# mike-gimelfarb/bboptpy

Measured on AMD Instinct MI355X. Metric: candidate-evals/sec, higher is better.
Workload: dtype f64; 1 GPU; ActiveCMAES n=128 np=4096 rosenbrock, 256 independent populations per GPU in lockstep; populations_per_gpu=256, n=128, np=4096, objective=rosenbrock

## Files before the change

### bboptpy_amd/csrc/bbo_cma.hip

```cpp
#include "bbo_cma_kernels.hpp"
#include "bbo_sep_kernels.hpp"
#include "bbo_chol_kernels.hpp"
#include "bbo_eig_mw.hpp"

#include <algorithm>
#include <atomic>
#include <cmath>
#include <cstdlib>
#include <limits>

namespace bbo {

namespace {

enum { K_SAMPLE = 0, K_RANK, K_WHITEN, K_GRAM, K_PATHS, K_COV, K_EIGEN, K_POST, K_STOP, K_COUNT };
static const char *const K_NAMES[K_COUNT] = { "bbo:cma_sample_eval", "bbo:cma_rank", "bbo:cma_whiten", "bbo:cma_gram", "bbo:cma_paths", "bbo:cma_cov", "bbo:cma_eigen", "bbo:cma_post", "bbo:cma_history_stop" };

int pick_maxt(int ld)
{
    const int per_wave = ((ld >> 4) + 3) / 4;
    if (per_wave <= 1) return 1;
    if (per_wave <= 2) return 2;
    if (per_wave <= 4) return 4;
    return 8;
// ... 487 lines not shown
    timer_.end(stream_);
    BBO_HIP(hipGetLastError());
    c_.use_zn = (zn_valid && !c.bound) ? 1 : 0;
}

void CmaEngine::launch_rank()
{
    const CmaConst &c = c_;
    rank_wrote_norms_ = false;
    timer_.begin(stream_, K_RANK);
    if (c.lambda <= 64 && c.lambda >= 2 && c.npop >= 4) {
        hipLaunchKernelGGL(cma_rank_wave, dim3((c.npop + 3) / 4), dim3(256), 0, stream_, d_, c_);
    } else if (c.lambda <= SORT_LDS_MAX && c.npop >= 4) {
        int m = 2;
        while (m < c.lambda) m <<= 1;
        allow_lds((const void*) cma_rank_sort, 128 * 1024);
        const size_t lds = rank_sort_merges(m, d_.dbg) ? (size_t) m * 24 : (size_t) std::max(m, 1024) * 12;
        hipLaunchKernelGGL(cma_rank_sort, dim3(c.npop), dim3(sort_threads(m)), lds, stream_, d_,
                c_, m);
        rank_wrote_norms_ = c.variant == 1 && c.use_zn && !basis_maybe_stale_;
    } else {
        if ((long) c.npop * ((c.lambda + 31) / 32) <= 256 && c.lambda >= 2048 && !(d_.dbg & (128 | 4096)))
            hipLaunchKernelGGL(cma_rank64, dim3((c.lambda + 3) / 4, c.npop), dim3(256), 0, stream_, d_, c_);
        else if ((long) c.npop * ((c.lambda + 31) / 32) <= 512 && c.lambda >= 512 && !(d_.dbg & 128))
            hipLaunchKernelGGL(cma_rank32, dim3((c.lambda + 7) / 8, c.npop), dim3(256), 0, stream_, d_, c_);
        else
            hipLaunchKernelGGL(cma_rank, dim3((c.lambda + 31) / 32, c.npop), dim3(256), 0, stream_, d_, c_);
        rank_wrote_norms_ = c.variant == 1 && c.use_zn && !basis_maybe_stale_;
    }
    timer_.end(stream_);
    BBO_HIP(hipGetLastError());
}

void CmaEngine::launch_update()
{
    const CmaConst &c = c_;
    if (c.variant == 3) {
        timer_.begin(stream_, K_PATHS);
        hipLaunchKernelGGL(chol_paths, dim3(c.npop), dim3(256), 0, stream_, d_, c_);
        timer_.end(stream_);
        const int NT = c.ld / 16;
        timer_.begin(stream_, K_GRAM);
        hipLaunchKernelGGL(chol_cprime, dim3(NT * (NT + 1) / 2, c.npop), dim3(256), 0, stream_, d_, c_);
        timer_.end(stream_);
        const int in_lds = c.ld <= 128 ? 1 : 0;
        const size_t lds = in_lds ? (size_t) c.ld * (c.ld + 1) * sizeof(double) : 0;
        timer_.begin(stream_, K_COV);
        hipLaunchKernelGGL(chol_factor, dim3(c.npop), dim3(256), lds, stream_, d_, c_, in_lds);
        timer_.end(stream_);
        BBO_HIP(hipGetLastError());
        return;
    }
    if (c.variant == 2) {
        timer_.begin(stream_, K_GRAM);
        hipLaunchKernelGGL(sep_moments, dim3(c.splits, (c.ld + 511) / 512, c.npop), dim3(256), 0,
                stream_, d_, c_);
        timer_.end(stream_);
        timer_.begin(stream_, K_PATHS);
        hipLaunchKernelGGL(sep_paths, dim3(c.npop), dim3(256), 0, stream_, d_, c_);
        timer_.end(stream_);
        BBO_HIP(hipGetLastError());
        return;
    }
    const bool norms_done = rank_wrote_norms_;
    rank_wrote_norms_ = false;
    if (c.variant == 1 && !norms_done) {
        timer_.begin(stream_, K_WHITEN);
// ... 18 lines not shown
        timer_.end(stream_);
        BBO_HIP(hipGetLastError());
    }
    if (c.ld == 128) {
        const size_t lds = (size_t) (2 * G128_CH * G128_LDY + 4 * G128_CH) * sizeof(double);
        allow_lds((const void*) cma_gram128, 80 * 1024);
        timer_.begin(stream_, K_GRAM);
        if (d_.dbg & 512)
            hipLaunchKernelGGL(cma_gram128, dim3(c.splits, c.npop), dim3(256), lds, stream_, d_, c_);
        else
            hipLaunchKernelGGL(cma_gram128s, dim3(c.splits, c.npop), dim3(256), 0, stream_, d_, c_);
        timer_.end(stream_);
        BBO_HIP(hipGetLastError());
    } else {
        const int NT = c.ld / 16, LT = NT * (NT + 1) / 2;
        const int ldy = gram_ldy(c.ld);
        dim3 grid(c.splits, (LT + 4 * GRAM_TPW - 1) / (4 * GRAM_TPW), c.npop);
        const size_t lds = gram_lds_bytes(c.ld, c.rps);
        allow_lds((const void*) cma_gram, (int) GRAM_LDS_MAX);
        timer_.begin(stream_, K_GRAM);
        hipLaunchKernelGGL(cma_gram, grid, dim3(256), lds, stream_, d_, c_, ldy);
        timer_.end(stream_);
        BBO_HIP(hipGetLastError());
    }
    timer_.begin(stream_, K_PATHS);
    if (c.lazy_isc && c.n >= 64 && !(d_.dbg & 131072))
        hipLaunchKernelGGL(cma_paths_lazy1k, dim3(c.npop), dim3(1024), 0, stream_, d_, c_);
    else if (c.lazy_isc)
        hipLaunchKernelGGL(cma_paths_lazy, dim3(c.npop), dim3(256), 0, stream_, d_, c_);
    else
        hipLaunchKernelGGL(cma_paths, dim3(c.npop), dim3(256), 0, stream_, d_, c_);
    timer_.end(stream_);
    BBO_HIP(hipGetLastError());
    {
        const int total = c.n * (c.n + 1) / 2;
        dim3 grid((total + 255) / 256, c.npop);
        timer_.begin(stream_, K_COV);
        hipLaunchKernelGGL(cma_cov, grid, dim3(256), 0, stream_, d_, c_);
        timer_.end(stream_);
        BBO_HIP(hipGetLastError());
    }
}

int CmaEngine::next_mw_xcd()
{
    static std::atomic<int> counter { 0 };
    return counter.fetch_add(1) & 7;
}

void CmaEngine::launch_eigen()
{
    const CmaConst &c = c_;
    if (c.variant >= 2) return;
    const EigPlan pl_lds = eig_plan(c.n, c.ld);
    const bool split128 = pl_lds.use_lds && pl_lds.threads == 512 && pl_lds.dc && c.npop <= split_maxp_
            && !(d_.dbg & (2 | 4 | 8 | 1024 | 4194304));
    const EigPlan pl = split128 ? eig_plan_split(c.n, c.ld) : pl_lds;
    bool wy4_packs = false, fcols_closed = false;
    allow_lds((const void*) cma_eigen, 160 * 1024 - 768);
    allow_lds((const void*) cma_eigen_g, 160 * 1024 - 768);
    allow_lds((const void*) cma_eigen_b, 160 * 1024 - 768);
    allow_lds((const void*) cma_eigen_256, 160 * 1024 - 768);
    allow_lds((const void*) cma_eigen_128, 160 * 1024 - 768);
    timer_.begin(stream_, K_EIGEN);
    const bool big_spread = c.n > 256 && pl.dc && !pl.hybrid && !mw_disabled_
            && !(d_.dbg & (2 | 16777216)) && mw_reserve((long) c.npop * 16);
    const bool small = c.n <= 16 && c.n >= 2 && c.ld == 16 && !(d_.dbg & 16);
    const int eig_path_bits = 1 | 2 | 4 | 8 | 1024 | 2048 | 8192 | 16384 | 32768 | 524288 | 2097152 | 4194304 | 8388608;
    const bool fixed_shape = c.n == 128 && c.ld == 128 && pl_lds.use_lds && pl_lds.dc && pl_lds.reg_path
            && pl_lds.threads == 512 && pl_lds.lda == EIG_FX_PLAN.lda && pl_lds.rc == EIG_FX_PLAN.rc
            && pl_lds.lds_bytes == EIG_FX_PLAN.lds_bytes && !d_.stamps && !(d_.dbg & eig_path_bits);
    const bool fixed128 = fixed_shape && c.npop > split_maxp_ && !split128 && c.lazy_isc;
    const bool fixed_r1 = fixed_shape && split128 && pl.hybrid;
    eig_fixed_last_ = (fixed128 || fixed_r1) && !small;
    if (small)
        hipLaunchKernelGGL(cma_eigen_small, dim3((c.npop + 3) / 4), dim3(256), 0, stream_, d_, c_, 0,
                1);
    else if (pl.threads == 128)
        hipLaunchKernelGGL(cma_eigen_128, dim3(c.npop), dim3(128), pl.lds_bytes, stream_, d_, c_,
                pl, 0);
    else if (pl.threads == 256)
        hipLaunchKernelGGL(cma_eigen_256, dim3(c.npop), dim3(256), pl.lds_bytes, stream_, d_, c_,
                pl, 0);
    else if (fixed128) {
        allow_lds((const void*) cma_eigen_fx128, 160 * 1024 - 768);
        const EigFxArgs fa { d_.C, d_.B, d_.D, d_.BDp, d_.eig_work, d_.scal, c.eigenfreq, c.honor_stop };
        hipLaunchKernelGGL(cma_eigen_fx128, dim3(c.npop), dim3(512), EIG_FX_PLAN.lds_bytes, stream_, fa);
    } else if (pl.use_lds)
        hipLaunchKernelGGL(cma_eigen, dim3(c.npop), dim3(512), pl.lds_bytes, stream_, d_, c_,
                pl, 0);
    else if (pl.hybrid && !(d_.dbg & (2 | 1024 | 4194304))) {
        const EigPlan plh = eig_plan(128, 128);
        allow_lds((const void*) cma_eigen_g1, 160 * 1024 - 768);
        allow_lds((const void*) cma_eigen_g2, 160 * 1024 - 768);
        allow_lds((const void*) cma_eig_halves, 160 * 1024 - 768);
        const bool use_mw = !split128 && !mw_disabled_ && !(d_.dbg & 16777216) && mw_reserve((long) c.npop * MW_G);
        if (split128 && fixed_r1) {
            allow_lds((const void*) cma_eigen_r1_fx128, 160 * 1024 - 768);
            const EigFxArgs fa { d_.C, d_.B, d_.D, d_.BDp, d_.eig_work, d_.scal, c.eigenfreq, c.honor_stop };
            hipLaunchKernelGGL(cma_eigen_r1_fx128, dim3(c.npop), dim3(512), EIG_FX_PLAN.lds_bytes, stream_, fa);
        } else if (split128) {
            allow_lds((const void*) cma_eigen_r1, 160 * 1024 - 768);
            hipLaunchKernelGGL(cma_eigen_r1, dim3(c.npop), dim3(512), pl_lds.lds_bytes, stream_, d_, c_,
                    pl_lds, 0);
        } else if (use_mw) {
            mw_launched_ = true;
            if (mw_buf_.count != (size_t) c.npop * MW_BUF_DOUBLES) mw_buf_.alloc((size_t) c.npop * MW_BUF_DOUBLES);
            const int istop = (d_.dbg & 536870912) ? 1 : 128;
            hipLaunchKernelGGL(cma_tred_mw, dim3(8 * MW_G, c.npop), dim3(MW_T), 0, stream_, d_, c_, 0,
                    mw_buf_.p, ++mw_launch_, istop, mw_xcd_);
            if (istop > 1) {
                allow_lds((const void*) cma_tred_tail, 160 * 1024 - 768);
                hipLaunchKernelGGL(cma_tred_tail, dim3(c.npop), dim3(512), pl.lds_bytes, stream_, d_, c_, pl, 0);
            }
        } else
            hipLaunchKernelGGL(cma_eigen_g1, dim3(c.npop), dim3(512), pl.lds_bytes, stream_, d_, c_, pl, 0);
        hipLaunchKernelGGL(cma_eig_halves, dim3(3, c.npop), dim3(512), plh.lds_bytes, stream_, d_, c_,
                plh, pl.lda);
        if ((long) c.npop * 8 <= 256 && !(d_.dbg & 67108864)) {
            hipLaunchKernelGGL(cma_eigen_g2, dim3(c.npop), dim3(512), pl.lds_bytes, stream_, d_, c_, pl, 1);
            hipLaunchKernelGGL(cma_eig_secular, dim3((c.n + 31) / 32, c.npop), dim3(512), 0, stream_, d_, c_);
            fcols_closed = !(c.n & 1) && c.lazy_isc && (long) c.npop * ((c.n + 15) / 16) <= 256
                    && !(d_.dbg & (33554432 | 134217728));
            if (fcols_closed) {
                hipLaunchKernelGGL(cma_eig_lowner, dim3((c.n + 31) / 32, c.npop), dim3(512), 0, stream_, d_, c_);
                hipLaunchKernelGGL(cma_eig_fcols, dim3((c.n + 31) / 32, c.npop), dim3(512), 0, stream_, d_, c_);
            } else
                hipLaunchKernelGGL(cma_eigen_g2, dim3(c.npop), dim3(512), pl.lds_bytes, stream_, d_, c_, pl, 2);
        } else
            hipLaunchKernelGGL(cma_eigen_g2, dim3(c.npop), dim3(512), pl.lds_bytes, stream_, d_, c_, pl, 0);
    } else if (pl.hybrid)
        hipLaunchKernelGGL(cma_eigen_g, dim3(c.npop), dim3(512), pl.lds_bytes, stream_, d_, c_,
// ... 90 lines not shown
    const CmaConst &c = c_;
    return c.variant < 2 && c.ld == 16 && c.n >= 2 && c.lambda_pad <= 64 && obj_.fused()
            && c.npop <= SMALL_FUSED_MAXP && !timer_.on() && !(d_.dbg & (16 | 64));
}

void CmaEngine::launch_small(int gens, bool honor_stop)
{
    c_.honor_stop = honor_stop ? 1 : 0;
    c_.use_zn = c_.bound ? 0 : 1;
    const int ldy = gram_ldy(c_.ld);
    size_t lds = gram_lds_bytes(c_.ld, c_.rps);
    lds = std::max(lds, (size_t) 64 * (c_.ld + 2) * sizeof(double));
    lds = std::max(lds, (size_t) (16 * (c_.ld + 2) + 64) * sizeof(double));
    const int scratch = (int) ((lds + 15) / 16 * 2);
    const size_t total = ((size_t) scratch + small_state_doubles(c_)) * sizeof(double);
    allow_lds((const void*) cma_small_generations, 120 * 1024);
    BBO_REQUIRE(total <= 120 * 1024, "small fused path: state does not fit LDS");
    hipLaunchKernelGGL(cma_small_generations, dim3(c_.npop), dim3(256), total, stream_, d_, c_,
            gens, ldy, scratch);
    BBO_HIP(hipGetLastError());
}

void CmaEngine::generation(bool honor_stop)
{
    if (small_fused_ok()) {
        launch_small(1, honor_stop);
        return;
    }
    c_.honor_stop = honor_stop ? 1 : 0;
    launch_sample_eval();
    if (obj_.needs_host()) host_evaluate();
    else if (obj_.is_program()) program_evaluate();
    launch_rank();
    launch_update();
    launch_eigen();
    launch_history_stop();
}

void CmaEngine::phase(int which)
{
    BBO_REQUIRE(inited_, "phase before init");
    BBO_HIP(hipSetDevice(params_.device));
    c_.honor_stop = 0;
    d_.mw_fault = mw_fault_from_env();
    switch (which) {
    case BBO_PHASE_SAMPLE_EVALUATE:
        launch_sample_eval();
        if (obj_.needs_host()) host_evaluate();
        else if (obj_.is_program()) program_evaluate();
        break;
    case BBO_PHASE_RANK: launch_rank(); break;
    case BBO_PHASE_UPDATE: launch_update(); break;
    case BBO_PHASE_EIGEN: launch_eigen(); break;
    case BBO_PHASE_HISTORY_STOP: launch_history_stop(); break;
    default: throw Error(BBO_ERR_ARG, "unknown CMA phase");
    }
    BBO_HIP(hipStreamSynchronize(stream_));
    if (mw_check_failed() && which == BBO_PHASE_EIGEN) {
        launch_eigen();
        BBO_HIP(hipStreamSynchronize(stream_));
    }
    timer_.collect();
    prog_timer_.collect();
}

void CmaEngine::inject_normals(const double *z, int count)
{
    BBO_REQUIRE(inited_, "inject_normals before init");
// ... 188 lines not shown
    if (k == "best_hist" || k == "kth_hist") {
        if (out && cap >= c.hlen)
            (k == "best_hist" ? hist_best_ : hist_kth_).download(out, c.hlen, (size_t) p * c.hlen);
        return c.hlen;
    }
    CmaScal s;
    scal_.download(&s, 1, p);
    if (k == "sigma") return o.one(s.sigma);
    if (k == "it") return o.one(s.it);
    if (k == "fev") return o.one(s.fev);
    if (k == "flag") return o.one(s.flag);
    if (k == "stop") return o.one(s.stop);
    if (k == "hsig") return o.one(s.hsig);
    if (k == "pslen") return o.one(s.pslen);
    if (k == "fbest") return o.one(s.fbest);
    if (k == "fworst") return o.one(s.fworst);
    if (k == "eigenlastev") return o.one(s.eigenlastev);
    if (k == "eigen_done") return o.one(s.eigen_done);
    if (k == "basis_ok") return o.one(s.basis_ok);
    if (k == "eig_stage") return o.one(s.eig_stage);
    if (k == "eig_mw_fail") return o.one(s.eig_mw_fail);
    if (k == "chol_repairs") {
        if (c.variant != 3) throw Error(BBO_ERR_KEY, "'chol_repairs' belongs to CholeskyCMAES");
        int r = 0;
        chol_repairs_.download(&r, 1, p);
        return o.one(r);
    }
    if (c.variant == 3 && k == "chol_tri") return o.one(chol_tri_ ? 1 : 0);
    if (c.variant == 3 && k == "stol") return o.one(c.stol);
    if (c.variant == 3 && k == "ranked") return o.one(c.ranked);
    if (k == "eig_mw_off") return o.one(mw_disabled_ ? 1 : 0);
    if (k == "eig_split_maxp") return o.one(split_maxp_);
    if (k == "eig_fixed128") return o.one(eig_fixed_last_ ? 1 : 0);
    if (k == "eig_mw_reserved") return o.one((double) mw_reserved_);
    if (k == "eig_mw_capacity") {
        MwBudget &b = MwBudget::get();
        std::lock_guard<std::mutex> lock(b.m);
        return o.one((double) b.capacity(params_.device));
    }
    if (k == "best_len") return o.one(s.hist_len);
    if (k == "best_buffer") return o.one(s.hist_head);
    if (k == "ibest") return o.one(s.ibw[0]);
    if (k == "n") return o.one(c.n);
    if (k == "lambda") return o.one(c.lambda);
    if (k == "mu") return o.one(c.mu);
    if (k == "mueff") return o.one(c.mueff);
    if (k == "cc") return o.one(c.cc);
    if (k == "cs") return o.one(c.cs);
    if (k == "c1") return o.one(c.c1);
    if (k == "cmu") return o.one(c.cmu);
    if (k == "cneg") return o.one(c.cneg);
    if (k == "alphaold") return o.one(c.alphaold);
    if (k == "cm") return o.one(c.cm);
    if (k == "ccov") return o.one(c.ccov);
    if (k == "damps") return o.one(c.damps);
    if (k == "chi") return o.one(c.chi);
    if (k == "eigenfreq") return o.one(c.eigenfreq);
    if (k == "hlen") return o.one(c.hlen);
    if (k == "ik") return o.one(c.ik);
    if (k == "mit") return o.one(c.mit);
    if (k == "mfev") return o.one(c.mfev);
    if (k == "sigma0") return o.one(c.sigma0);
    throw Error(BBO_ERR_KEY, "unknown state key '" + k + "'");
}

int CmaEngine::set(const std::string &k, int p, const double *in, int count)
// ... 147 lines not shown
```

### bboptpy_amd/csrc/bbo_cma.hpp

```cpp
#pragma once

#include "bbo_engine.hpp"

namespace bbo {

struct CmaScal {
    double sigma;
    double fbest, fworst;
    double pslen;
    double ybw[4];
    int ibw[4];
    int it, fev;
    int flag;
    int stop;
    int hsig;
    int eigenlastev, eigen_done;
    int hist_head, hist_len;
    int basis_ok;
    int eig_stage;
    int eig_mw_fail;
};

struct CmaConst {
    int n, ld;
// ... 59 lines not shown
    void optimize(int n, const double *lower, const double *upper, const double *guess,
            const ObjectiveSpec &obj, double *x_out, int *n_evals, int *converged) override;
    int get(const std::string &key, int population, double *out, int cap) override;
    int set(const std::string &key, int population, const double *in, int count) override;
    int dimension() const override { return c_.n; }

    void set_params(int np, double sigma, int mfev);
    void phase(int which);
    void inject_normals(const double *z, int count);
    double evaluate_point(const double *x);
    int lambda() const { return params_.np; }
    int populations() const { return params_.populations; }
    uint64_t seed() const { return params_.seed; }
    void set_seed(uint64_t s) { params_.seed = s; }
    void fresh_start(uint64_t s)
    {
        params_.seed = s;
        keep_bc_ = false;
    }

private:
    static const bbo_params &checked(const bbo_params &p);
    void generation(bool honor_stop) override;
    bool budget_spent(const CmaScal &s) const override { return s.fev >= c_.mfev; }
    void inspect(const std::vector<CmaScal> &sc) override;
    int chunk_limit(int want) override;
    void launch_chunk(int gens) override;
    void after_chunk(bool in_run) override;
    bool small_fused_ok() const;
    void launch_small(int gens, bool honor_stop);
    void launch_sample_eval();
    void launch_post(int mode);
    void launch_rank();
    void launch_update();
    void launch_eigen();
    void launch_history_stop();
    void host_evaluate();
    void program_evaluate();

    CmaConst c_ {};
    CmaDev d_ {};
    bool keep_bc_ = false;
    bool basis_maybe_stale_ = false;
    DevBuf<double> mw_buf_;
    unsigned long long mw_launch_ = 0;
    bool mw_disabled_ = false;
    int mw_xcd_ = next_mw_xcd();
    static int next_mw_xcd();
    long sample_wide_max_tiles_ = 512;
    long sample128_min_rows_ = 256 * 128;
    bool chol_tri_ = true;
    int split_maxp_ = 32;
    bool eig_fixed_last_ = false;
    bool rank_wrote_norms_ = false;
    int last_n_ = -1;

    DevBuf<double> zn2_, csep_, A_;
    DevBuf<double> X_, f_, xmean_, xold_, pc_, ps_, C_, B_, D_, isc_, BDp_, ISp_, S_,
            gram_part_, mean_part_, hist_best_, hist_kth_, eig_work_, weights_, zinject_, zrecord_;
    DevBuf<int> rank_, order_, chol_repairs_;
    DevBuf<long long> stamps_;
    int *mw_fail_host_ = nullptr;
    long mw_reserved_ = 0;
    bool mw_launched_ = false;
    bool mw_reserve(long workgroups);
    void mw_release();
    bool mw_check_failed();
};

}
```

### bboptpy_amd/csrc/bbo_cma_kernels.hpp

```cpp
#pragma once

#include "bbo_cma.hpp"
#include "bbo_objectives.hpp"
#include "bbo_rng.hpp"
#include "bbo_eig.hpp"
#include "bbo_rank.hpp"

namespace bbo {

typedef double d4_t __attribute__((ext_vector_type(4)));

#define BBO_INF (__builtin_huge_val())

__device__ inline void cma_draw_quad(const CmaDev &d, const CmaConst &c, int p, int row, int q,
        int gen, uint32_t sw, const double2 *tab, double (&z)[4])
{
    const int j0 = cma_quad_col0(q);
    z[0] = z[1] = z[2] = z[3] = 0.;
    if (row < c.lambda && j0 < c.n) {
        if (d.zinject) {
            const double *zi = d.zinject + ((size_t) p * c.lambda + row) * c.n;
#pragma unroll
            for (int i = 0; i < 4; i++)
                if (j0 + 4 * i < c.n) z[i] = zi[j0 + 4 * i];
// ... 1344 lines not shown
        if (sc->it >= c.hlen && sc->fworst - sc->fbest == 0.) sg *= exp(0.2 + c.cs / c.damps);
        sc->sigma = sg;
        sc->hsig = hsig;
        sc->pslen = pslen;
    }
}

__global__ __launch_bounds__(256) void cma_paths(CmaDev d, CmaConst c)
{
    paths_body<false>(d, c, blockIdx.x);
}
__global__ __launch_bounds__(256) void cma_paths_lazy(CmaDev d, CmaConst c)
{
    paths_body<true>(d, c, blockIdx.x);
}
__global__ __launch_bounds__(1024) void cma_paths_lazy1k(CmaDev d, CmaConst c)
{
    paths_body<true, 1024>(d, c, blockIdx.x);
}

__device__ __forceinline__ void cov_body(const CmaDev &d, const CmaConst &c, int p, int bx)
{
    const CmaScal *sc = d.scal + p;
    if (pop_frozen(c, sc)) return;
    const int q = bx * 256 + threadIdx.x;
    const int total = c.n * (c.n + 1) / 2;
    if (q >= total) return;
    int i, j;
    tri_tile(q, i, j);
    const int ld = c.ld;
    double *C = d.C + (size_t) p * ld * ld;
    const double *pc = d.pc + (size_t) p * ld;
    const double cij = C[(size_t) i * ld + j];
    const double c2 = (1. - sc->hsig) * c.cc * (2. - c.cc);
    const double decay = c.variant == 1 ? (1. - c.c1 - c.cmu + c.cneg * c.alphaold)
                                        : (1. - c.c1 - c.cmu);
    double sum = decay * cij + c.c1 * (pc[i] * pc[j] + c2 * cij);
    const double *G = d.gram_part + (size_t) p * c.splits * ld * ld + (size_t) i * ld + j;
    double g = 0.;
    {
        int s = 0;
        for (; s + 8 <= c.splits; s += 8) {
            double x[8];
#pragma unroll
            for (int u = 0; u < 8; u++) x[u] = G[(size_t) (s + u) * ld * ld];
            __builtin_amdgcn_sched_barrier(0);
#pragma unroll
            for (int u = 0; u < 8; u++) g += x[u];
        }
        for (; s < c.splits; s++) g += G[(size_t) s * ld * ld];
    }
    sum += g;
    C[(size_t) i * ld + j] = sum;
    C[(size_t) j * ld + i] = sum;
}

__global__ __launch_bounds__(256) void cma_cov(CmaDev d, CmaConst c)
{
    cov_body(d, c, blockIdx.y, blockIdx.x);
}

__global__ __launch_bounds__(256) void cma_post(CmaDev d, CmaConst c, int mode)
{
    const int p = blockIdx.z;
    const CmaScal *sc = d.scal + p;
    if (pop_frozen(c, sc)) return;
    if (mode == 0 && !sc->eigen_done) return;
    if (mode == 3 && !sc->basis_ok) return;
    const bool gemm = mode == 3 || (mode != 2 && !c.lazy_isc);
    const int ld = c.ld, n = c.n;
// ... 521 lines not shown
```

### bboptpy_amd/csrc/bbo_eig.hpp

```cpp
#pragma once

#include <type_traits>

#include "bbo_cma.hpp"
#include "bbo_eig_ql.hpp"
#include "bbo_eig_dc.hpp"

namespace bbo {

typedef double d4_eig __attribute__((ext_vector_type(4)));

constexpr int EIG_THREADS = 512;
constexpr int EIG_NMAX = 512;

struct EigPlan {
    int threads;
    int use_lds;
    int reg_path;
    int dc;
    int hybrid;
    int lda;
    int rc;
    int vl;
    size_t lds_bytes;
// ... 34 lines not shown
        if (rc > cap) rc = cap;
        pl.rc = (int) rc;
        pl.lds_bytes = fixed + mat + (size_t) 2 * pl.rc * 16;
    } else {
        pl.use_lds = 0;
        pl.lda = (n + 31) & ~31;
        if (pl.hybrid) {
            pl.rc = 0;
            pl.lds_bytes = fixed + (size_t) 128 * 130 * sizeof(double);
        } else {
            pl.rc = 2048;
            pl.lds_bytes = fixed + (size_t) 2 * pl.rc * 16;
        }
    }
    return pl;
}

inline EigPlan eig_plan_split(int n, int ld)
{
    EigPlan pl = eig_plan(n, ld);
    pl.threads = EIG_THREADS;
    pl.vl = 128 + 2;
    pl.reg_path = 0;
    pl.hybrid = 1;
    pl.use_lds = 0;
    pl.lda = (n + 31) & ~31;
    pl.rc = 0;
    const size_t ints = (size_t) (2 * EIG_MAXSEQ * 3 + 8) * sizeof(int);
    const size_t vecs = ((size_t) EIG_NVEC * pl.vl + eig_part_doubles(pl.vl, false, true)) * sizeof(double);
    pl.lds_bytes = vecs + ints + (size_t) 128 * 130 * sizeof(double);
    return pl;
}

template<int AMAX>
__device__ inline double tred_matvec(const double (&a_)[4][8], double (&ur)[4][8], const double *uv,
        int q)
{
#pragma unroll
    for (int a = 0; a < AMAX; a++)
#pragma unroll
        for (int b = 0; b < 8; b += 2) {
            const double2 t2 = *reinterpret_cast<const double2*>(&uv[32 * a + 8 * q + b]);
            ur[a][b] = t2.x;
            ur[a][b + 1] = t2.y;
        }
    double acc0 = 0., acc1 = 0.;
#pragma unroll
    for (int a = 0; a < AMAX; a++)
#pragma unroll
        for (int b = 0; b < 8; b += 2) {
            acc0 = __builtin_fma(a_[a][b], ur[a][b], acc0);
            acc1 = __builtin_fma(a_[a][b + 1], ur[a][b + 1], acc1);
        }
    double acc = acc0 + acc1;
    acc = eig_quad_sum(acc);
    return acc;
}

template<int AMAX>
__device__ inline void tred_rank2(double (&a_)[4][8], const double (&ur)[4][8], const double *wv,
        double uj, double wj, int q)
{
#pragma unroll
    for (int a0 = 0; a0 < AMAX; a0 += 2) {
        double2 w2[2][4];
#pragma unroll
// ... 764 lines not shown
    }
#undef EIG_SEQ
#undef EIG_LDS_BARRIER
    __syncthreads();
}

__device__ inline void eig_tred_sym256(const double *C, int ld, int n, const EigMat &A,
        double *dv, double *ev, double *uv, double *wv, double *gv, double *hvec, double *td,
        int nv, int tid, long long *stamps, const EigMat &As, bool accumulate, double *Vout)
{
    constexpr int T = EIG_THREADS, LB = 130;
    const int nr = (n + 31) & ~31;
    eig_tred_sym256_steps(C, ld, n, A.a, A.ld, nv, stamps);
    if (stamps && tid == 0) stamps[2] = wall_clock64();
    eig_tred_accum_reg128(As.a, LB, 128, As, dv, ev, uv, wv, gv, hvec, td, tid, nullptr,
            A.a, A.ld, false, accumulate);
    for (int k = tid; k < nr; k += T) {
        uv[k] = 0.;
        wv[k] = 0.;
    }
    __syncthreads();
    const int lda = A.ld;
    for (int q = tid; q < n * n; q += T) {
        const int r = q / n, cidx = q - r * n;
        double v = 0.;
        if (cidx < r) v = r < 128 ? As(r, cidx) : A.a[(size_t) r * lda + cidx];
        Vout[q] = v;
    }
    __syncthreads();
    for (int k = tid; k < n; k += T) dv[k] = td[k];
    __syncthreads();
}

template<int TT, bool LDSM, int HYB = 1, int STAGE = 0, bool FX = false>
__device__ __forceinline__ void cma_eigen_impl(const CmaDev &d, const CmaConst &c, const EigPlan &pl,
        int force)
{
    const int p = blockIdx.x;
    CmaScal *sc = d.scal + p;
    if (c.honor_stop && sc->stop != 0) return;
    if (STAGE == 2 || STAGE == 4) {
        if (sc->eig_stage != 1) return;
    } else if (STAGE == 3) {
    } else
    if (!force && !((double) (sc->fev - sc->eigenlastev) > c.eigenfreq)) {
        if (threadIdx.x == 0) {
            sc->eigen_done = 0;
            sc->eig_stage = 0;
        }
        return;
    }
    extern __shared__ __attribute__((aligned(16))) double lds[];
    const int tid = threadIdx.x, T = TT, lane = tid & 63, wave = tid >> 6;
    const int n = c.n, ld = c.ld, nv = LDSM ? 130 : pl.vl;
    double *dv = lds + 2;
    double *ev = dv + nv;
    double *uv = ev + nv;
    double *wv = uv + nv;
    double *gv = wv + nv;
    double *hvec = gv + nv;
    double *td = hvec + nv;
    double *uh0 = td + nv, *uh1 = uh0 + nv;
    double *part = uh1 + nv - 2;
    double2 *rot = reinterpret_cast<double2*>(part
            + eig_part_doubles(nv, pl.reg_path != 0, pl.hybrid != 0));
    int *ibuf = reinterpret_cast<int*>(rot + 2 * pl.rc);
    int *desc = ibuf;
    int *nseq = ibuf + 2 * EIG_MAXSEQ * 3;
    int *sdone = nseq + 2;
    int *perm = reinterpret_cast<int*>(uv);
    EigMat A { LDSM ? reinterpret_cast<double*>(ibuf + 2 * EIG_MAXSEQ * 3 + 8)
                    : d.eig_work + (size_t) p * 4 * eig_slab(ld), pl.lda };
    double *C = d.C + (size_t) p * ld * ld;

#define EIG_STAMP(slot) do { if (d.stamps && p == 0 && tid == 0) d.stamps[slot] = wall_clock64(); } while (0)
    EIG_STAMP(0);
    if (tid < 2) {
        dv[-1 - tid] = 0.;
        ev[-1 - tid] = 0.;
    }
    double *tri = d.eig_work + (size_t) (4 * p + 3) * eig_slab(ld);
    if (STAGE == 3) {
        if (tri[4 * n + 1] != (force ? 2. : 1.) || sc->eig_mw_fail) return;
        constexpr int LB = 130;
        EigMat Ast { reinterpret_cast<double*>(ibuf + 2 * EIG_MAXSEQ * 3 + 8), LB };
        const double *L11 = d.eig_work + (size_t) (4 * p) * eig_slab(ld);
        for (int q = tid; q < 128 * 64; q += T) {
            const int r = q >> 6, c2 = (q & 63) * 2;
            *reinterpret_cast<double2*>(&Ast.a[r * LB + c2]) =
                    *reinterpret_cast<const double2*>(&L11[(size_t) r * 128 + c2]);
        }
        __syncthreads();
        eig_tred_accum_reg128(Ast.a, LB, 128, Ast, dv, ev, uv, wv, gv, hvec, td, tid, nullptr, A.a, A.ld,
                false, false);
        double *Vout = d.eig_work + (size_t) (4 * p + 1) * eig_slab(ld);
        for (int i = tid; i < 128; i += T) {
            tri[i] = td[i];
            if (i >= 1) tri[n + i - 1] = ev[i];
            tri[2 * n + i] = hvec[i];
        }
        for (int r = wave; r < 128; r += T / 64)
            for (int cidx = lane; cidx < n; cidx += 64) Vout[(size_t) r * n + cidx] = cidx < r ? Ast(r, cidx) : 0.;
        if (tid == 0) sc->eig_stage = 1;
        return;
    }
    if (STAGE == 2 || STAGE == 4) {
        for (int i = tid; i < n; i += T) {
            dv[i] = STAGE == 2 ? tri[3 * n + i] : tri[i];
            ev[i] = tri[n + i];
            hvec[i] = tri[2 * n + i];
        }
        __syncthreads();
    } else {
    if (LDSM) {
        eig_tred_accum_reg128<TT>(C, ld, n, A, dv, ev, uv, wv, gv, hvec, td, tid,
                (d.stamps && p == 0) ? d.stamps : nullptr, A.a, A.ld, true,
                !(pl.dc && !(d.dbg & 2)));
    } else if (TT == EIG_THREADS && !LDSM) {
        const bool hybrid = HYB != 0;
        EigMat Ast { reinterpret_cast<double*>(ibuf + 2 * EIG_MAXSEQ * 3 + 8), 128 };
        if (hybrid && !(d.dbg & 2) && !(d.dbg & 1024))
            eig_tred_sym256(C, ld, n, A, dv, ev, uv, wv, gv, hvec, td, nv, tid,
                    (d.stamps && p == 0) ? d.stamps : nullptr, Ast, false,
                    d.eig_work + (size_t) (4 * p + 1) * eig_slab(ld));
        else
        eig_tred_accum_global(C, ld, n, A, dv, ev, uv, wv, gv, hvec, td, part, nv, tid,
                (d.stamps && p == 0) ? d.stamps : nullptr, hybrid ? &Ast : nullptr,
                !(hybrid && !(d.dbg & 2)));
    }
    {
        const double t = (tid + 1 < n) ? ev[tid + 1] : 0.;
        __syncthreads();
        if (tid < n) ev[tid] = t;
    }
    __syncthreads();
    }
    EIG_STAMP(3);
    if (STAGE == 1 || STAGE == 5) {
        for (int i = tid; i < n; i += T) {
            tri[i] = dv[i];
            tri[n + i] = ev[i];
            tri[2 * n + i] = hvec[i];
        }
        if (STAGE == 5) {
            double *Vout = d.eig_work + (size_t) (4 * p + 1) * eig_slab(ld);
            for (int r = wave; r < n; r += T / 64)
                for (int cidx = lane; cidx < n; cidx += 64) Vout[(size_t) r * n + cidx] = A(r, cidx);
// ... 114 lines not shown
        for (int j = tid; j < n; j += T) dv[j] = sqrt(gv[j]);
        __syncthreads();
        double *BDp = d.BDp + (size_t) p * ld * ld;
        const int KS = ld >> 2;
        for (int q = tid; q < ld * ld; q += T) {
            const int t4 = q >> 6, l = q & 63;
            const int nt = t4 / KS, ks = t4 - nt * KS;
            const int i = nt * 16 + (l & 15), j = 4 * ks + (l >> 4);
            BDp[q] = (i < n && j < n) ? A(i, j) * dv[j] : 0.;
        }
        if (tid == 0) sc->basis_ok = 1;
    }
    EIG_STAMP(5);
#undef EIG_STAMP
}

__global__ __launch_bounds__(512) void cma_eigen(CmaDev d, CmaConst c, EigPlan pl, int force)
{
    cma_eigen_impl<512, true>(d, c, pl, force);
}
__global__ __launch_bounds__(512) void cma_eigen_g(CmaDev d, CmaConst c, EigPlan pl, int force)
{
    cma_eigen_impl<512, false, 1>(d, c, pl, force);
}
__global__ __launch_bounds__(512) void cma_eigen_b(CmaDev d, CmaConst c, EigPlan pl, int force)
{
    cma_eigen_impl<512, false, 0>(d, c, pl, force);
}
struct EigFxArgs {
    double *C, *B, *D, *BDp, *eig_work;
    CmaScal *scal;
    double eigenfreq;
    int honor_stop;
};
constexpr EigPlan EIG_FX_PLAN = eig_plan(128, 128);
__global__ __launch_bounds__(512) void cma_eigen_fx128(EigFxArgs a)
{
    static_assert(EIG_FX_PLAN.use_lds == 1 && EIG_FX_PLAN.dc == 1 && EIG_FX_PLAN.reg_path == 1
            && EIG_FX_PLAN.threads == 512 && EIG_FX_PLAN.vl == 130, "cma_eigen_fx128: the plan of n = 128");
    CmaDev d {};
    d.C = a.C;
    d.B = a.B;
    d.D = a.D;
    d.BDp = a.BDp;
    d.eig_work = a.eig_work;
    d.scal = a.scal;
    CmaConst c {};
    c.n = c.ld = 128;
    c.lazy_isc = 1;
    c.honor_stop = a.honor_stop;
    c.eigenfreq = a.eigenfreq;
    cma_eigen_impl<512, true, 1, 0, true>(d, c, EIG_FX_PLAN, 0);
}
__global__ __launch_bounds__(512) void cma_eigen_r1_fx128(EigFxArgs a)
{
    CmaDev d {};
    d.C = a.C;
    d.eig_work = a.eig_work;
    d.scal = a.scal;
    CmaConst c {};
    c.n = c.ld = 128;
    c.honor_stop = a.honor_stop;
    c.eigenfreq = a.eigenfreq;
    cma_eigen_impl<512, true, 1, 5, true>(d, c, EIG_FX_PLAN, 0);
}
__global__ __launch_bounds__(512) void cma_eigen_g1(CmaDev d, CmaConst c, EigPlan pl, int force)
{
    cma_eigen_impl<512, false, 1, 1>(d, c, pl, force);
}
__global__ __launch_bounds__(512) void cma_eigen_r1(CmaDev d, CmaConst c, EigPlan pl, int force)
{
    cma_eigen_impl<512, true, 1, 5>(d, c, pl, force);
}
__global__ __launch_bounds__(512) void cma_eigen_b4(CmaDev d, CmaConst c, EigPlan pl, int force)
{
    cma_eigen_impl<512, false, 0, 4>(d, c, pl, force);
}
__global__ __launch_bounds__(512) void cma_tred_tail(CmaDev d, CmaConst c, EigPlan pl, int chained)
{
    cma_eigen_impl<512, false, 1, 3>(d, c, pl, chained);
}
__global__ __launch_bounds__(512) void cma_eigen_g2(CmaDev d, CmaConst c, EigPlan pl, int part)
{
    cma_eigen_impl<512, false, 1, 2>(d, c, pl, part);
}
// ... 741 lines not shown
```

Baseline: 713.0 million candidate-evals/s.

## Fuse covariance update into fixed n=128 eigen kernel prologue

```diff
diff --git a/bboptpy_amd/csrc/bbo_cma.hip b/bboptpy_amd/csrc/bbo_cma.hip
--- a/bboptpy_amd/csrc/bbo_cma.hip
+++ b/bboptpy_amd/csrc/bbo_cma.hip
@@ -543,7 +543,7 @@
     BBO_HIP(hipGetLastError());
 }
 
-void CmaEngine::launch_update()
+void CmaEngine::launch_update(bool with_cov)
 {
     const CmaConst &c = c_;
     if (c.variant == 3) {
@@ -628,7 +628,7 @@
         hipLaunchKernelGGL(cma_paths, dim3(c.npop), dim3(256), 0, stream_, d_, c_);
     timer_.end(stream_);
     BBO_HIP(hipGetLastError());
-    {
+    if (with_cov) {
         const int total = c.n * (c.n + 1) / 2;
         dim3 grid((total + 255) / 256, c.npop);
         timer_.begin(stream_, K_COV);
@@ -644,9 +644,26 @@
     return counter.fetch_add(1) & 7;
 }
 
-void CmaEngine::launch_eigen()
+int CmaEngine::eig_fixed_form() const
 {
     const CmaConst &c = c_;
+    if (c.variant >= 2 || c.n != 128 || c.ld != 128) return 0;
+    const EigPlan pl_lds = eig_plan(c.n, c.ld);
+    const bool split128 = pl_lds.use_lds && pl_lds.threads == 512 && pl_lds.dc && c.npop <= split_maxp_
+            && !(d_.dbg & (2 | 4 | 8 | 1024 | 4194304));
+    const int eig_path_bits = 1 | 2 | 4 | 8 | 1024 | 2048 | 8192 | 16384 | 32768 | 524288 | 2097152 | 4194304 | 8388608;
+    const bool fixed_shape = pl_lds.use_lds && pl_lds.dc && pl_lds.reg_path
+            && pl_lds.threads == 512 && pl_lds.lda == EIG_FX_PLAN.lda && pl_lds.rc == EIG_FX_PLAN.rc
+            && pl_lds.lds_bytes == EIG_FX_PLAN.lds_bytes && !d_.stamps && !(d_.dbg & eig_path_bits);
+    if (fixed_shape && c.npop > split_maxp_ && !split128 && c.lazy_isc) return 1;
+    if (fixed_shape && split128 && eig_plan_split(c.n, c.ld).hybrid) return 2;
+    return 0;
+}
+
+void CmaEngine::launch_eigen(bool cov_fused)
+{
+    const CmaConst &c = c_;
+    cov_fused_last_ = false;
     if (c.variant >= 2) return;
     const EigPlan pl_lds = eig_plan(c.n, c.ld);
     const bool split128 = pl_lds.use_lds && pl_lds.threads == 512 && pl_lds.dc && c.npop <= split_maxp_
@@ -662,13 +679,13 @@
     const bool big_spread = c.n > 256 && pl.dc && !pl.hybrid && !mw_disabled_
             && !(d_.dbg & (2 | 16777216)) && mw_reserve((long) c.npop * 16);
     const bool small = c.n <= 16 && c.n >= 2 && c.ld == 16 && !(d_.dbg & 16);
-    const int eig_path_bits = 1 | 2 | 4 | 8 | 1024 | 2048 | 8192 | 16384 | 32768 | 524288 | 2097152 | 4194304 | 8388608;
-    const bool fixed_shape = c.n == 128 && c.ld == 128 && pl_lds.use_lds && pl_lds.dc && pl_lds.reg_path
-            && pl_lds.threads == 512 && pl_lds.lda == EIG_FX_PLAN.lda && pl_lds.rc == EIG_FX_PLAN.rc
-            && pl_lds.lds_bytes == EIG_FX_PLAN.lds_bytes && !d_.stamps && !(d_.dbg & eig_path_bits);
-    const bool fixed128 = fixed_shape && c.npop > split_maxp_ && !split128 && c.lazy_isc;
-    const bool fixed_r1 = fixed_shape && split128 && pl.hybrid;
-    eig_fixed_last_ = (fixed128 || fixed_r1) && !small;
+    const int fixed_form = eig_fixed_form();
+    const bool fixed128 = fixed_form == 1, fixed_r1 = fixed_form == 2;
+    eig_fixed_last_ = fixed_form != 0;
+    BBO_REQUIRE(!cov_fused || fixed128, "C is formed by cma_eigen_fx128 only");
+    cov_fused_last_ = cov_fused;
+    const EigFxArgs fa { d_.C, d_.B, d_.D, d_.BDp, d_.eig_work, d_.scal, c.eigenfreq, c.honor_stop,
+            c.splits, c.variant, d_.gram_part, d_.pc, c.cc, c.c1, c.cmu, c.cneg, c.alphaold };
     if (small)
         hipLaunchKernelGGL(cma_eigen_small, dim3((c.npop + 3) / 4), dim3(256), 0, stream_, d_, c_, 0,
                 1);
@@ -680,8 +697,11 @@
                 pl, 0);
     else if (fixed128) {
         allow_lds((const void*) cma_eigen_fx128, 160 * 1024 - 768);
-        const EigFxArgs fa { d_.C, d_.B, d_.D, d_.BDp, d_.eig_work, d_.scal, c.eigenfreq, c.honor_stop };
-        hipLaunchKernelGGL(cma_eigen_fx128, dim3(c.npop), dim3(512), EIG_FX_PLAN.lds_bytes, stream_, fa);
+        allow_lds((const void*) cma_eigen_fx128u, 160 * 1024 - 768);
+        if (cov_fused)
+            hipLaunchKernelGGL(cma_eigen_fx128, dim3(c.npop), dim3(512), EIG_FX_PLAN.lds_bytes, stream_, fa);
+        else
+            hipLaunchKernelGGL(cma_eigen_fx128u, dim3(c.npop), dim3(512), EIG_FX_PLAN.lds_bytes, stream_, fa);
     } else if (pl.use_lds)
         hipLaunchKernelGGL(cma_eigen, dim3(c.npop), dim3(512), pl.lds_bytes, stream_, d_, c_,
                 pl, 0);
@@ -693,7 +713,6 @@
         const bool use_mw = !split128 && !mw_disabled_ && !(d_.dbg & 16777216) && mw_reserve((long) c.npop * MW_G);
         if (split128 && fixed_r1) {
             allow_lds((const void*) cma_eigen_r1_fx128, 160 * 1024 - 768);
-            const EigFxArgs fa { d_.C, d_.B, d_.D, d_.BDp, d_.eig_work, d_.scal, c.eigenfreq, c.honor_stop };
             hipLaunchKernelGGL(cma_eigen_r1_fx128, dim3(c.npop), dim3(512), EIG_FX_PLAN.lds_bytes, stream_, fa);
         } else if (split128) {
             allow_lds((const void*) cma_eigen_r1, 160 * 1024 - 768);
@@ -850,8 +869,9 @@
     if (obj_.needs_host()) host_evaluate();
     else if (obj_.is_program()) program_evaluate();
     launch_rank();
-    launch_update();
-    launch_eigen();
+    const bool fuse_cov = eig_fixed_form() == 1 && !(d_.dbg & 32);
+    launch_update(!fuse_cov);
+    launch_eigen(fuse_cov);
     launch_history_stop();
 }
 
@@ -1106,6 +1126,8 @@
     if (k == "eig_mw_off") return o.one(mw_disabled_ ? 1 : 0);
     if (k == "eig_split_maxp") return o.one(split_maxp_);
     if (k == "eig_fixed128") return o.one(eig_fixed_last_ ? 1 : 0);
+    if (k == "cov_fused") return o.one(cov_fused_last_ ? 1 : 0);
+    if (k == "splits") return o.one(c.splits);
     if (k == "eig_mw_reserved") return o.one((double) mw_reserved_);
     if (k == "eig_mw_capacity") {
         MwBudget &b = MwBudget::get();
diff --git a/bboptpy_amd/csrc/bbo_cma.hpp b/bboptpy_amd/csrc/bbo_cma.hpp
--- a/bboptpy_amd/csrc/bbo_cma.hpp
+++ b/bboptpy_amd/csrc/bbo_cma.hpp
@@ -115,8 +115,9 @@
     void launch_sample_eval();
     void launch_post(int mode);
     void launch_rank();
-    void launch_update();
-    void launch_eigen();
+    void launch_update(bool with_cov = true);
+    void launch_eigen(bool cov_fused = false);
+    int eig_fixed_form() const;
     void launch_history_stop();
     void host_evaluate();
     void program_evaluate();
@@ -135,6 +136,7 @@
     bool chol_tri_ = true;
     int split_maxp_ = 32;
     bool eig_fixed_last_ = false;
+    bool cov_fused_last_ = false;
     bool rank_wrote_norms_ = false;
     int last_n_ = -1;
 
diff --git a/bboptpy_amd/csrc/bbo_cma_kernels.hpp b/bboptpy_amd/csrc/bbo_cma_kernels.hpp
--- a/bboptpy_amd/csrc/bbo_cma_kernels.hpp
+++ b/bboptpy_amd/csrc/bbo_cma_kernels.hpp
@@ -1400,10 +1400,8 @@
     double *C = d.C + (size_t) p * ld * ld;
     const double *pc = d.pc + (size_t) p * ld;
     const double cij = C[(size_t) i * ld + j];
-    const double c2 = (1. - sc->hsig) * c.cc * (2. - c.cc);
-    const double decay = c.variant == 1 ? (1. - c.c1 - c.cmu + c.cneg * c.alphaold)
-                                        : (1. - c.c1 - c.cmu);
-    double sum = decay * cij + c.c1 * (pc[i] * pc[j] + c2 * cij);
+    const CovCoef k = cov_coef(c, sc->hsig);
+    double sum = cov_elem(k, cij, pc[i], pc[j]);
     const double *G = d.gram_part + (size_t) p * c.splits * ld * ld + (size_t) i * ld + j;
     double g = 0.;
     {
diff --git a/bboptpy_amd/csrc/bbo_eig.hpp b/bboptpy_amd/csrc/bbo_eig.hpp
--- a/bboptpy_amd/csrc/bbo_eig.hpp
+++ b/bboptpy_amd/csrc/bbo_eig.hpp
@@ -90,6 +90,21 @@
     return pl;
 }
 
+struct CovCoef {
+    double c1, c2, decay;
+};
+__device__ __forceinline__ CovCoef cov_coef(const CmaConst &c, int hsig)
+{
+    const double c2 = (1. - hsig) * c.cc * (2. - c.cc);
+    const double decay = c.variant == 1 ? (1. - c.c1 - c.cmu + c.cneg * c.alphaold)
+                                        : (1. - c.c1 - c.cmu);
+    return CovCoef { c.c1, c2, decay };
+}
+__device__ __forceinline__ double cov_elem(const CovCoef &k, double cij, double pci, double pcj)
+{
+    return k.decay * cij + k.c1 * (pci * pcj + k.c2 * cij);
+}
+
 template<int AMAX>
 __device__ inline double tred_matvec(const double (&a_)[4][8], double (&ur)[4][8], const double *uv,
         int q)
@@ -920,13 +935,97 @@
     __syncthreads();
 }
 
-template<int TT, bool LDSM, int HYB = 1, int STAGE = 0, bool FX = false>
+template<int TT>
+__device__ inline void eig_cov_prologue128(const CmaDev &d, const CmaConst &c, const CmaScal *sc, int p,
+        double *As, int tid)
+{
+    constexpr int N = 128, LB = eig_plan(128, 128).lda, EPT = 12;
+    double *C = d.C + (size_t) p * N * N;
+    const int lane = tid & 63, wave = __builtin_amdgcn_readfirstlane(tid >> 6);
+    const double *pc = d.pc + (size_t) p * N;
+    const int splits = c.splits;
+    const double *G = d.gram_part + (size_t) p * splits * N * N;
+    const CovCoef k = cov_coef(c, sc->hsig);
+    const double pcl0 = pc[lane], pcl1 = pc[lane + 64];
+    static_assert(24 % EPT == 0, "eig_cov_prologue128: 24 elements per thread");
+#pragma unroll
+    for (int e0 = 0; e0 < 24; e0 += EPT) {
+        int off[EPT];
+        bool ok[EPT];
+        double cij[EPT], pci[EPT], g[EPT];
+#pragma unroll
+        for (int u = 0; u < EPT; u++) {
+            const int e = e0 + u;
+            const int i = e < 8 ? wave + 8 * e : 64 + wave + 8 * ((e - 8) >> 1);
+            const int j = e < 8 ? lane : lane + 64 * ((e - 8) & 1);
+            ok[u] = j <= i;
+            off[u] = i * N + j;
+            cij[u] = ok[u] ? C[off[u]] : 0.;
+            pci[u] = pc[i];
+            g[u] = 0.;
+        }
+        int s = 0;
+        for (; s + 4 <= splits; s += 4) {
+            double x[4][EPT];
+#pragma unroll
+            for (int u = 0; u < EPT; u++)
+#pragma unroll
+                for (int v = 0; v < 4; v++) x[v][u] = ok[u] ? G[(size_t) (s + v) * N * N + off[u]] : 0.;
+#pragma unroll
+            for (int u = 0; u < EPT; u++)
+#pragma unroll
+                for (int v = 0; v < 4; v++) g[u] += x[v][u];
+        }
+        if (s + 2 <= splits) {
+            double x0[EPT], x1[EPT];
+#pragma unroll
+            for (int u = 0; u < EPT; u++) {
+                x0[u] = ok[u] ? G[(size_t) s * N * N + off[u]] : 0.;
+                x1[u] = ok[u] ? G[(size_t) (s + 1) * N * N + off[u]] : 0.;
+            }
+#pragma unroll
+            for (int u = 0; u < EPT; u++) {
+                g[u] += x0[u];
+                g[u] += x1[u];
+            }
+            s += 2;
+        }
+        if (s < splits) {
+            double x0[EPT];
+#pragma unroll
+            for (int u = 0; u < EPT; u++) x0[u] = ok[u] ? G[(size_t) s * N * N + off[u]] : 0.;
+#pragma unroll
+            for (int u = 0; u < EPT; u++) g[u] += x0[u];
+        }
+#pragma unroll
+        for (int u = 0; u < EPT; u++) {
+            const int e = e0 + u;
+            const int i = e < 8 ? wave + 8 * e : 64 + wave + 8 * ((e - 8) >> 1);
+            const int h = e < 8 ? 0 : ((e - 8) & 1);
+            const int j = lane + 64 * h;
+            double sum = cov_elem(k, cij[u], pci[u], h ? pcl1 : pcl0);
+            sum += g[u];
+            if (ok[u]) {
+                As[i * LB + j] = sum;
+                As[j * LB + i] = sum;
+            }
+        }
+    }
+    __syncthreads();
+    for (int q = tid; q < N * (N / 2); q += TT) {
+        const int r = q >> 6, c2 = (q & 63) * 2;
+        *reinterpret_cast<double2*>(&C[r * N + c2]) = make_double2(As[r * LB + c2], As[r * LB + c2 + 1]);
+    }
+}
+
+template<int TT, bool LDSM, int HYB = 1, int STAGE = 0, bool FX = false, bool PRO = false>
 __device__ __forceinline__ void cma_eigen_impl(const CmaDev &d, const CmaConst &c, const EigPlan &pl,
         int force)
 {
     const int p = blockIdx.x;
     CmaScal *sc = d.scal + p;
     if (c.honor_stop && sc->stop != 0) return;
+    bool due = true;
     if (STAGE == 2 || STAGE == 4) {
         if (sc->eig_stage != 1) return;
     } else if (STAGE == 3) {
@@ -936,7 +1035,8 @@
             sc->eigen_done = 0;
             sc->eig_stage = 0;
         }
-        return;
+        if (!PRO) return;
+        due = false;
     }
     extern __shared__ __attribute__((aligned(16))) double lds[];
     const int tid = threadIdx.x, T = TT, lane = tid & 63, wave = tid >> 6;
@@ -1000,7 +1100,12 @@
         }
         __syncthreads();
     } else {
-    if (LDSM) {
+    if (PRO) {
+        eig_cov_prologue128<TT>(d, c, sc, p, A.a, tid);
+        if (!due) return;
+        eig_tred_accum_reg128<TT>(A.a, A.ld, n, A, dv, ev, uv, wv, gv, hvec, td, tid, nullptr, A.a, A.ld, true,
+                !(pl.dc && !(d.dbg & 2)));
+    } else if (LDSM) {
         eig_tred_accum_reg128<TT>(C, ld, n, A, dv, ev, uv, wv, gv, hvec, td, tid,
                 (d.stamps && p == 0) ? d.stamps : nullptr, A.a, A.ld, true,
                 !(pl.dc && !(d.dbg & 2)));
@@ -1181,9 +1286,25 @@
     CmaScal *scal;
     double eigenfreq;
     int honor_stop;
+    int splits, variant;
+    const double *gram_part, *pc;
+    double cc, c1, cmu, cneg, alphaold;
 };
+__device__ __forceinline__ void eig_fx_cov_args(const EigFxArgs &a, CmaDev &d, CmaConst &c)
+{
+    d.gram_part = const_cast<double*>(a.gram_part);
+    d.pc = const_cast<double*>(a.pc);
+    c.splits = a.splits;
+    c.variant = a.variant;
+    c.cc = a.cc;
+    c.c1 = a.c1;
+    c.cmu = a.cmu;
+    c.cneg = a.cneg;
+    c.alphaold = a.alphaold;
+}
 constexpr EigPlan EIG_FX_PLAN = eig_plan(128, 128);
-__global__ __launch_bounds__(512) void cma_eigen_fx128(EigFxArgs a)
+template<bool PRO>
+__device__ __forceinline__ void cma_eigen_fx128_body(const EigFxArgs &a)
 {
     static_assert(EIG_FX_PLAN.use_lds == 1 && EIG_FX_PLAN.dc == 1 && EIG_FX_PLAN.reg_path == 1
             && EIG_FX_PLAN.threads == 512 && EIG_FX_PLAN.vl == 130, "cma_eigen_fx128: the plan of n = 128");
@@ -1199,7 +1320,16 @@
     c.lazy_isc = 1;
     c.honor_stop = a.honor_stop;
     c.eigenfreq = a.eigenfreq;
-    cma_eigen_impl<512, true, 1, 0, true>(d, c, EIG_FX_PLAN, 0);
+    if (PRO) eig_fx_cov_args(a, d, c);
+    cma_eigen_impl<512, true, 1, 0, true, PRO>(d, c, EIG_FX_PLAN, 0);
+}
+__global__ __launch_bounds__(512) void cma_eigen_fx128(EigFxArgs a)
+{
+    cma_eigen_fx128_body<true>(a);
+}
+__global__ __launch_bounds__(512) void cma_eigen_fx128u(EigFxArgs a)
+{
+    cma_eigen_fx128_body<false>(a);
 }
 __global__ __launch_bounds__(512) void cma_eigen_r1_fx128(EigFxArgs a)
 {
```

Measured after the change: 722.7 million candidate-evals/s, median of 6. +1.4%, better.
